# madsjulia/GeostatInversion.jl

Hardware: AMD Instinct MI355X
Metric: randSVD GB/s + top-k singular-value rel-err, n=1e6 rank=256 (higher is better)
Workload: dtype f64

## Files before the change

geostatinversion.jl_amd/_lib.py:

```python
import ctypes as C
import os

import numpy as np

_HERE = os.path.dirname(os.path.abspath(__file__))
LIB_PATH = os.path.join(_HERE, "libgsi_hip.so")

GSI_OK = 0
ERR_NAMES = {1: "GSI_ERR_ARG", 2: "GSI_ERR_NEG_ITERS", 3: "GSI_ERR_SINGULAR", 4: "GSI_ERR_HIP",
             5: "GSI_ERR_RCCL", 6: "GSI_ERR_OOM", 7: "GSI_ERR_NOT_POSDEF", 8: "GSI_ERR_INTERNAL"}
PHASES = ["gemm_n", "gemm_t", "lu", "qr", "svd", "small_gemm", "comm", "other", "comm_wait"]
UNIQUE_ID_BYTES = 128

c_i64 = C.c_int64
c_dp = C.POINTER(C.c_double)
c_vp = C.c_void_p
RANDN_FN = C.CFUNCTYPE(None, c_vp, c_dp, c_i64)

SIGNATURES = {
    "gsi_version": (C.c_int, []),
    "gsi_last_error": (C.c_char_p, []),
    "gsi_backend_name": (C.c_char_p, []),
    "gsi_ctx_create": (C.c_int, [C.POINTER(c_vp), C.c_int]),
    "gsi_ctx_destroy": (C.c_int, [c_vp]),
# ... 28 lines not shown
    "gsi_randsvd": (C.c_int, [c_vp, c_vp, c_dp, c_i64, c_i64, c_i64, c_dp, c_dp]),
    "gsi_randsvd_dense_host": (C.c_int, [c_vp, c_dp, c_i64, c_i64, c_i64, c_dp, c_i64, c_i64, c_i64, c_dp, c_dp, C.POINTER(c_vp)]),
    "gsi_rangefinder_dense_host": (C.c_int, [c_vp, c_dp, c_i64, c_i64, c_i64, c_dp, c_i64, c_i64, c_dp, C.POINTER(c_vp)]),
    "gsi_eig_nystrom": (C.c_int, [c_vp, c_vp, c_dp, c_i64, c_dp, c_dp]),
    "gsi_rangefinder_adaptive": (C.c_int, [c_vp, c_vp, RANDN_FN, c_vp, C.c_double, c_i64, c_dp, C.POINTER(c_i64)]),
    "gsi_mat_create": (C.c_int, [c_vp, C.POINTER(c_vp), c_i64, c_i64]),
    "gsi_mat_destroy": (C.c_int, [c_vp]),
    "gsi_mat_upload": (C.c_int, [c_vp, c_vp, c_dp, c_i64]),
    "gsi_mat_download": (C.c_int, [c_vp, c_vp, c_dp, c_i64]),
    "gsi_mat_randn": (C.c_int, [c_vp, c_vp, C.c_uint64]),
    "gsi_op_mul_dev": (C.c_int, [c_vp, c_vp, C.c_int, c_vp, c_vp]),
    "gsi_rangefinder_dev": (C.c_int, [c_vp, c_vp, c_vp, c_i64, c_vp]),
    "gsi_randsvd_dev": (C.c_int, [c_vp, c_vp, c_vp, c_i64, c_i64, c_i64, c_vp, c_vp]),
    "gsi_randsvd_rows": (C.c_int, [c_vp, c_vp, c_vp, c_i64, c_i64, c_i64, c_vp, c_vp]),
    "gsi_lu_L": (C.c_int, [c_vp, c_dp, c_i64, c_i64, c_dp, C.POINTER(C.c_int32)]),
    "gsi_lu_L_dev": (C.c_int, [c_vp, c_vp, C.POINTER(C.c_int32)]),
    "gsi_lu_L_sharded": (C.c_int, [c_vp, c_dp, c_i64, c_i64, c_dp, C.POINTER(C.c_int32)]),
    "gsi_lu_L_sharded_virtual": (C.c_int, [c_vp, c_dp, c_i64, c_i64, C.c_int, c_dp, C.POINTER(C.c_int32)]),
    "gsi_qr_thinQ": (C.c_int, [c_vp, c_dp, c_i64, c_i64, c_dp, c_dp]),
    "gsi_svd_tall": (C.c_int, [c_vp, c_dp, c_i64, c_i64, c_dp, c_dp]),
    "gsi_gemm": (C.c_int, [c_vp, C.c_int, c_i64, c_i64, c_i64, C.c_double, c_dp, c_i64, c_dp, c_i64, c_dp, c_i64]),
    "gsi_gemm_view": (C.c_int, [c_vp, C.c_int, C.c_int, c_i64, c_i64, c_i64, C.c_double, C.c_double, c_dp, c_i64, c_i64,
                                c_dp, c_i64, c_i64, c_dp, c_i64, c_i64, c_i64, c_i64, C.POINTER(c_i64)]),
    "gsi_pcga_params": (C.c_int, [c_vp, c_dp, c_i64, c_i64, c_dp, c_dp, C.c_double, c_dp]),
    "gsi_pcga_update": (C.c_int, [c_vp, c_dp, c_i64, c_i64, c_dp, C.c_double, c_dp, c_i64, c_dp, c_dp]),
    "gsi_pcga_params_dev": (C.c_int, [c_vp, c_vp, c_i64, c_dp, c_dp, C.c_double, c_dp]),
    "gsi_pcga_update_dev": (C.c_int, [c_vp, c_vp, c_i64, c_dp, C.c_double, c_dp, c_i64, c_dp, c_dp]),
    "gsi_mat_download_col": (C.c_int, [c_vp, c_vp, c_i64, c_dp]),
    "gsi_op_lowrank_solve": (C.c_int, [c_vp, c_vp, c_dp, c_dp, C.POINTER(c_i64)]),
    "gsi_pcgamat_create": (C.c_int, [c_vp, C.POINTER(c_vp), c_dp, c_i64, c_i64, c_dp, c_dp, C.c_int]),
    "gsi_pcgamat_destroy": (C.c_int, [c_vp]),
    "gsi_pcgamat_mul": (C.c_int, [c_vp, c_vp, c_dp, c_dp]),
    "gsi_pcgamat_lsqr": (C.c_int, [c_vp, c_vp, c_dp, c_dp, C.POINTER(c_i64)]),
    "gsi_basis_create": (C.c_int, [c_vp, C.POINTER(c_vp), c_vp, c_i64, C.c_int]),
    "gsi_basis_destroy": (C.c_int, [c_vp]),
    "gsi_pcga_params_basis": (C.c_int, [c_vp, c_vp, c_dp, c_dp, C.c_double, c_dp]),
    "gsi_pcga_update_basis": (C.c_int, [c_vp, c_vp, c_dp, C.c_double, c_dp, c_i64, c_dp, c_dp]),
    "gsi_basis_download_col": (C.c_int, [c_vp, c_vp, c_i64, c_dp]),
    "gsi_ctx_profile": (C.c_int, [c_vp, C.c_int]),
    "gsi_ctx_phase_reset": (C.c_int, [c_vp]),
    "gsi_ctx_phase_times": (C.c_int, [c_vp, c_dp, C.POINTER(c_i64)]),
    "gsi_ctx_counters": (C.c_int, [c_vp, C.POINTER(c_i64)]),
    "gsi_ctx_path_info": (C.c_int, [c_vp, C.POINTER(c_i64), c_i64]),
    "gsi_ctx_pinned_copy_rate": (C.c_int, [c_vp, c_i64, c_dp, c_dp]),
    "gsi_ctx_release_cache": (C.c_int, [c_vp]),
    "gsi_ctx_device_bytes": (C.c_int, [c_vp, C.POINTER(c_i64)]),
# ... 50 lines not shown
```

geostatinversion.jl_amd/csrc/api.cpp:

```cpp
#include <cmath>
#include <cstdlib>
#include <cstring>
#include <memory>
#include <new>
#include <string>
#include <vector>
#include "../../include/gsi_hip.h"
#include "pipeline.hpp"
#include "pointcov.hpp"

using namespace gsi;

struct gsi_ctx {
  Context c;
};
struct gsi_op {
  Operator op;
};
struct gsi_mat {
  gsi_ctx* ctx;
  Buf buf;
  int64_t rows, cols;
  int refs = 1;
};
// ... 944 lines not shown
    REQUIRE(form != 1 || m == l, "gemm_view: form 1 is the l x l product A'A (m == l)");
    REQUIRE(form != 3 || (r0 >= 0 && r0 + m <= m_full), "gemm_view: row block outside the full product");
    const bool tn = trans || form == 1;
    const int64_t ar = (form == 3) ? m_full : (tn ? k : m), ac = tn ? m : k;
    const int64_t crows = (form == 3) ? m_full : m;
    REQUIRE(lda >= ar && ldc >= crows && (form == 1 || ldb >= k), "leading dimension too small");
    REQUIRE(a_off >= 0 && b_off >= 0 && c_off >= 0, "negative offset");
    Backend* be = ctx->c.be.get();
    const size_t na = (size_t)a_off + (size_t)lda * (size_t)ac, nc = (size_t)c_off + (size_t)ldc * (size_t)l;
    const size_t nb = (form == 1) ? 1 : (size_t)b_off + (size_t)ldb * (size_t)l;
    Buf Ad(be, na), Bd(be, nb), Cd(be, nc);
    be->fill_bytes(Ad.p, 0xFF, na);
    be->fill_bytes(Bd.p, 0xFF, nb);
    be->upload2d(Ad.p + a_off, lda, A, ar, ar, ac);
    if (form != 1) be->upload2d(Bd.p + b_off, ldb, B, k, k, l);
    be->upload2d(Cd.p, (int64_t)nc, C, (int64_t)nc, (int64_t)nc, 1);
    be->gemm_view(form, trans != 0, m, l, k, alpha, Ad.p + a_off, lda, Bd.p + b_off, ldb, beta, Cd.p + c_off, ldc, m_full, r0,
                  plan_out);
    be->download2d(C, (int64_t)nc, Cd.p, (int64_t)nc, (int64_t)nc, 1);
    check_async_errors(ctx->c);
  });
}

namespace {
void pcga_params_impl(Context& c, const double* Zdev, int64_t n, int64_t K, const double* s, const double* X,
                      double delta, double* out) {
  Backend* be = c.be.get();
  Buf O(be, (size_t)n * (K + 3)), sv(be, (size_t)n), Xv(be, (size_t)n);
  be->upload2d(sv.p, n, s, n, n, 1);
  be->upload2d(Xv.p, n, X, n, n, 1);
  be->pcga_params(Zdev, n, K, sv.p, Xv.p, delta, O.p);
  be->download2d(out, n, O.p, n, n, K + 3);
}
void pcga_update_impl(Context& c, const double* Zdev, int64_t n, int64_t K, const double* X, double beta_bar,
                      const double* etas, int64_t nobs, const double* xi_bar, double* s_out) {
  Backend* be = c.be.get();
  Buf E(be, (size_t)nobs * K), xb(be, (size_t)nobs), w(be, (size_t)K), sd(be, (size_t)n), Xd(be, (size_t)n);
  be->upload2d(E.p, nobs, etas, nobs, nobs, K);
  be->upload2d(xb.p, nobs, xi_bar, nobs, nobs, 1);
  be->upload2d(Xd.p, n, X, n, n, 1);
  be->gemm_tn(K, 1, nobs, 1.0, E.p, nobs, xb.p, nobs, 0.0, w.p, K);
  be->scal_copy(n, beta_bar, Xd.p, sd.p);
  be->gemm_nn(n, 1, K, 1.0, Zdev, n, w.p, K, 1.0, sd.p, n);
  be->download2d(s_out, n, sd.p, n, n, 1);
}
}
// ... 246 lines not shown
```

geostatinversion.jl_amd/csrc/backend.hpp:

```cpp
#pragma once
#include <cstddef>
#include <cstdint>
#include <stdexcept>
#include <string>

namespace gsi {

struct Error : std::runtime_error {
  int code;
  Error(int c, const std::string& msg) : std::runtime_error(msg), code(c) {}
};

enum Phase : int {
  PH_GEMM_N = 0, PH_GEMM_T = 1, PH_LU = 2, PH_QR = 3, PH_SVD = 4, PH_SMALL_GEMM = 5,
  PH_COMM = 6, PH_OTHER = 7, PH_COMM_WAIT = 8, PH_COUNT = 9
};

class Backend {
 public:
  virtual ~Backend() {}
  virtual const char* name() const = 0;

  virtual double* alloc(size_t count) = 0;
  virtual void release(double* p) = 0;
// ... 11 lines not shown
    upload2d(dst, ldd, host, ldh, rows, cols);
    return nullptr;
  }
  virtual void pinned_copy_rate(int64_t bytes, double* h2d_gbs, double* d2h_gbs) { (void)bytes; *h2d_gbs = 0.0; *d2h_gbs = 0.0; }
  virtual void upload2d_wait_block(void* handle, int64_t b) { (void)handle; (void)b; }
  virtual void upload2d_end(void* handle) { (void)handle; }

  virtual void gemm_nn(int64_t m, int64_t l, int64_t k, double alpha, const double* A, int64_t lda,
                       const double* B, int64_t ldb, double beta, double* C, int64_t ldc) = 0;
  virtual void gemm_nn_rowblock(int64_t m_full, int64_t r0, int64_t mb, int64_t l, int64_t k, const double* A, int64_t lda,
                                const double* B, int64_t ldb, double* C, int64_t ldc) {
    (void)m_full;
    gemm_nn(mb, l, k, 1.0, A + r0, lda, B, ldb, 0.0, C + r0, ldc);
  }
  virtual void gemm_tn(int64_t m, int64_t l, int64_t k, double alpha, const double* A, int64_t lda,
                       const double* B, int64_t ldb, double beta, double* C, int64_t ldc) = 0;

  virtual void gemm_view(int form, bool trans, int64_t m, int64_t l, int64_t k, double alpha, const double* A, int64_t lda,
                         const double* B, int64_t ldb, double beta, double* C, int64_t ldc, int64_t m_full, int64_t r0,
                         int64_t* plan8) {
    (void)form; (void)trans; (void)m; (void)l; (void)k; (void)alpha; (void)A; (void)lda; (void)B; (void)ldb; (void)beta;
    (void)C; (void)ldc; (void)m_full; (void)r0; (void)plan8;
    throw Error(1 , "gemm_view: not available on this backend");
  }
  virtual void fill_bytes(double* p, int byte, size_t count) {
    (void)p; (void)byte; (void)count;
    throw Error(1 , "fill_bytes: not available on this backend");
  }

  virtual void gemm_nn_gridcov(int64_t m, int64_t l, int64_t k, const double* tab, int64_t nx, int64_t ny,
                               int64_t roff, int64_t koff, const double* B, int64_t ldb, double* C,
                               int64_t ldc) = 0;

  virtual void gemm_nn_pointcov(int64_t m, int64_t l, int64_t k, const double* pts, int d, int kind, double ell,
                                double sigma2, double nugget, int64_t roff, int64_t koff, const double* B, int64_t ldb,
                                double* C, int64_t ldc) = 0;

  virtual void* fftcov_create(const int64_t N[3], double beta, int fftrf) = 0;
  virtual void* fftcov_create_lags(const int64_t N[3], int kind, const double ell[3], double theta, double sigma2,
                                   double nugget, const double* table, const double* table_mirror) {
    (void)N; (void)kind; (void)ell; (void)theta; (void)sigma2; (void)nugget; (void)table; (void)table_mirror;
    throw Error(1 , "fft covariance from a covariance function or table: not supported by this backend");
  }
  virtual void fftcov_destroy(void* plan) = 0;
  virtual void fftcov_apply(void* plan, int64_t l, const double* X, int64_t ldx, double* Y, int64_t ldy) = 0;

// ... 170 lines not shown
```

geostatinversion.jl_amd/csrc/cholqr.hip:

```cpp
#include "hip_common.hpp"
#include <atomic>
#include <cfloat>
#include <cstdio>
#include <cstdlib>

namespace gsi { namespace hipk {

constexpr int CQ_TB = 32;

__global__ __launch_bounds__(256) void cq_diagmax_kernel(const double* __restrict__ G, int l, double* __restrict__ tiny) {
  __shared__ double s[256];
  double mx = 0.0;
  for (int i = threadIdx.x; i < l; i += 256) mx = fmax(mx, G[i + (int64_t)i * l]);
  s[threadIdx.x] = mx;
  __syncthreads();
  for (int st = 128; st > 0; st >>= 1) {
    if (threadIdx.x < st) s[threadIdx.x] = fmax(s[threadIdx.x], s[threadIdx.x + st]);
    __syncthreads();
  }
  if (threadIdx.x == 0) tiny[0] = s[0] * (double)l * DBL_EPSILON * 16.0;
}

__device__ __forceinline__ double cq_bcast(double v, int src) {
  const int lo = __builtin_amdgcn_readlane(__double2loint(v), src);
// ... 205 lines not shown
    for (int j = 0; j < 8; ++j) {
#pragma unroll
      for (int i = 0; i < j; ++i) acc[j] -= Ds[(pb + i) * CQF_DS + pb + j] * acc[i];
      acc[j] *= Dinv[pb + j];
    }
#pragma unroll
    for (int j = 0; j < 8; ++j) {
      const double v = (pb + j < b) ? acc[j] : 0.0;
      us[(pb + j) * CQF_LDU] = v;
      if constexpr (!VEC) { if (pb + j < b) gcol[pb + j] = v; }
    }
    if constexpr (VEC) {
      double2* o2 = reinterpret_cast<double2*>(gcol + pb);
#pragma unroll
      for (int j = 0; j < 8; j += 2) o2[j >> 1] = make_double2(acc[j], acc[j + 1]);
    }
    asm volatile("" ::: "memory");
  }
}
#define CQF_STAMP(ph) do { if (trace != nullptr && tid == 0) { const unsigned long long now_ = wall_clock64(); trace[ph] += now_ - t_last; t_last = now_; } } while (0)
__device__ __forceinline__ void cqf_tri_inverse(const double* __restrict__ G, int l, double* __restrict__ X, double* Us,
                                                double* Ds, int tid, int lane, int wave, unsigned long long* trace,
                                                unsigned long long& t_last);
__global__ __launch_bounds__(CQF_THREADS) void cq_chol_inv_kernel(double* __restrict__ G, int l, double* __restrict__ X,
                                                                  int32_t* __restrict__ flag, unsigned long long* __restrict__ trace) {
  unsigned long long t_last = (trace != nullptr) ? wall_clock64() : 0ull;
  extern __shared__ double cqf_lds[];
  double* Us = cqf_lds;
  double* Ds = Us + CQ_TB * CQF_LDU;
  double* Dinv = Ds + CQ_TB * CQF_DS;
  double* red = Dinv + CQ_TB;
  const int tid = threadIdx.x, lane = tid & 63, wave = tid >> 6;
  const int nblk = (l + CQ_TB - 1) / CQ_TB;
  {
    double mx = 0.0;
    for (int i = tid; i < l; i += CQF_THREADS) mx = fmax(mx, G[i + (int64_t)i * l]);
    for (int off = 32; off > 0; off >>= 1) mx = fmax(mx, __shfl_xor(mx, off, 64));
    if (lane == 0) red[wave] = mx;
    __syncthreads();
    if (tid == 0) {
      double m2 = 0.0;
      for (int w2 = 0; w2 < CQF_THREADS / 64; ++w2) m2 = fmax(m2, red[w2]);
      red[32] = m2 * (double)l * DBL_EPSILON * 16.0;
    }
    for (int64_t e = tid; e < (int64_t)l * l; e += CQF_THREADS) X[e] = 0.0;
    __syncthreads();
  }
  const double tiny = red[32];
  CQF_STAMP(0);

  auto trailing_tiles = [&](int j0, int b, int nc, int ncp, bool first_rows, int w0, int nw) __attribute__((always_inline)) {
    const int nt = ncp >> 4;
    const int nfirst = (nt >= 2) ? (2 * nt - 1) : nt;
    const int ntot = nt * (nt + 1) / 2;
    const int cnt = first_rows ? nfirst : ntot - nfirst;
    const int base = first_rows ? 0 : nfirst;
    const int jl = lane & 15, kq = lane >> 4;
    double* Gt = G + (int64_t)(j0 + b) + (int64_t)(j0 + b) * l;
    constexpr int TPP = 4;
    if (wave < w0 || wave >= w0 + nw) return;
    for (int t0 = wave - w0; t0 < cnt; t0 += nw * TPP) {
      cq_double4 acc[TPP];
      int trs[TPP], tcs[TPP];
#pragma unroll
      for (int u = 0; u < TPP; ++u) {
        const int tl = t0 + u * nw;
        int tr = 0, rem = base + ((tl < cnt) ? tl : 0);
        while (rem >= nt - tr) { rem -= nt - tr; ++tr; }
// ... 42 lines not shown
        else cqf_block_row_col<false>(G + j0 + (int64_t)(j0 + b + c) * l, b, Ds, Dinv, Us + c);
      } else {
#pragma unroll
        for (int p = 0; p < CQ_TB; ++p) Us[p * CQF_LDU + c] = 0.0;
      }
    }
    for (int e = tid; e < b * nc; e += CQF_THREADS) {
      const int r = j0 + b + e % nc, c = j0 + e / nc;
      G[r + (int64_t)c * l] = 0.0;
    }
    __syncthreads();
    CQF_STAMP(2);
    trailing_tiles(j0, b, nc, ncp, true, 0, CQF_THREADS / 64);
    __syncthreads();
    {
      const int j1 = j0 + b;
      const int b1 = (l - j1 < CQ_TB) ? (l - j1) : CQ_TB;
      if (wave == 0) cqf_chol_diag(G, l, j1, b1, tiny, Ds, Dinv, flag, lane);
      trailing_tiles(j0, b, nc, ncp, false, 1, CQF_THREADS / 64 - 1);
    }
    __syncthreads();
    CQF_STAMP(3);
  }
  cqf_tri_inverse(G, l, X, Us, Ds, tid, lane, wave, trace, t_last);
}

__device__ __forceinline__ void cqf_tri_inverse(const double* __restrict__ G, int l, double* __restrict__ X, double* Us,
                                                double* Ds, int tid, int lane, int wave, unsigned long long* trace,
                                                unsigned long long& t_last) {
  const int nblk = (l + CQ_TB - 1) / CQ_TB;
  for (int jb = wave; jb < nblk; jb += CQF_THREADS / 64) {
    const int j0 = jb * CQ_TB;
    cqf_inv_diag(G, l, j0, (l - j0 < CQ_TB) ? (l - j0) : CQ_TB, X, lane);
  }
  __syncthreads();
  CQF_STAMP(4);
  double* Wt = Us;
  double* Xjj = Ds;
  for (int jb = 1; jb < nblk; ++jb) {
    const int j0 = jb * CQ_TB;
    const int b = (l - j0 < CQ_TB) ? (l - j0) : CQ_TB;
    for (int e = tid; e < CQ_TB * CQ_TB; e += CQF_THREADS) {
      const int r = e & (CQ_TB - 1), c = e >> 5;
      Xjj[r * CQF_DS + c] = (r < b && c < b) ? X[(j0 + r) + (int64_t)(j0 + c) * l] : 0.0;
    }
    __syncthreads();
    {
// ... 181 lines not shown
  const int l = (int)l64;
  const CqBufs b = cq_bufs(small, l);
  if (!trmm_upper_tall(st, m, l, T, ldt, b.X2, l, Y, ld)) gemm_f64_trmm_upper(st, m, l, l, T, ldt, b.X2, l, Y, ld, gemm_ws);
  if (R != nullptr)
    hipLaunchKernelGGL(cq_triprod_kernel, dim3(grid_for((int64_t)l * l, 256)), dim3(256), 0, st, b.R2, b.R1, l, R);
}

void cholqr2_R(hipStream_t st, int64_t l64, double* small, double* R) {
  const int l = (int)l64;
  const CqBufs b = cq_bufs(small, l);
  hipLaunchKernelGGL(cq_triprod_kernel, dim3(grid_for((int64_t)l * l, 256)), dim3(256), 0, st, b.R2, b.R1, l, R);
}
const double* cholqr2_X2(const double* small, int64_t l) { return small + 5 * (size_t)l * (size_t)l; }

void mirror_upper(hipStream_t st, double* G, int64_t l) {
  hipLaunchKernelGGL(cq_mirror_upper_kernel, dim3(64), dim3(256), 0, st, G, (int)l);
}
bool cq_gram_round(hipStream_t st, double* Gm, int64_t l64, double* X, bool check, int32_t* flag) {
  const int l = (int)l64;
  if (l < 1 || l > CQF_MAXL) return false;
  hipLaunchKernelGGL(cq_mirror_upper_kernel, dim3(64), dim3(256), 0, st, Gm, l);
  if (check)
    hipLaunchKernelGGL(cq_orth_check_kernel, dim3(grid_for((int64_t)l * l, 64)), dim3(256), 0, st, Gm, l, 0.1, flag);
  static std::atomic<uint64_t> attr_mask{0};
  if (first_use_on_this_device(attr_mask))
    (void)hipFuncSetAttribute((const void*)cq_chol_inv_kernel, hipFuncAttributeMaxDynamicSharedMemorySize, (int)CQF_LDS_BYTES);
  hipLaunchKernelGGL(cq_chol_inv_kernel, dim3(1), dim3(CQF_THREADS), CQF_LDS_BYTES, st, Gm, l, X, flag,
                     (unsigned long long*)nullptr);
  return true;
}
void tri_product(hipStream_t st, const double* R2, const double* R1, int64_t l, double* R) {
  hipLaunchKernelGGL(cq_triprod_kernel, dim3(grid_for(l * l, 256)), dim3(256), 0, st, R2, R1, (int)l, R);
}

__global__ __launch_bounds__(256) void lr_gather_rows_kernel(const double* __restrict__ S, int64_t lds, int64_t N,
                                                             const int64_t* __restrict__ src, const int64_t* __restrict__ sub,
                                                             int64_t nr, double* __restrict__ R, int64_t ldr) {
  const int64_t total = nr * N;
  for (int64_t e = (int64_t)blockIdx.x * blockDim.x + threadIdx.x; e < total; e += (int64_t)gridDim.x * blockDim.x) {
    const int64_t k = e % nr, c = e / nr;
    const double* col = S + c * lds;
    const int64_t s = sub[k];
    double v = col[src[k]];
    if (s >= 0) v -= col[s];
    R[k + c * ldr] = v;
  }
// ... 60 lines not shown
```

geostatinversion.jl_amd/csrc/hip_backend.hip:

```cpp
#include <hip/hip_runtime.h>
#include <rccl/rccl.h>
#include <dlfcn.h>
#include <fcntl.h>
#include <sched.h>
#include <sys/mman.h>
#include <time.h>
#include <unistd.h>
#include <algorithm>
#include <cmath>
#include <cstdlib>
#include <cstring>
#include <condition_variable>
#include <atomic>
#include <mutex>
#include <string>
#include <chrono>
#include <map>
#include <memory>
#include <set>
#include <vector>
#include "../../include/gsi_hip.h"
#include "backend.hpp"
#include "hip_common.hpp"
#include "host_staging.hpp"
// ... 311 lines not shown
    check_launch("gemm_tn");
  }
  void gemm_view(int form, bool trans, int64_t m, int64_t l, int64_t k, double alpha, const double* A, int64_t lda,
                 const double* B, int64_t ldb, double beta, double* C, int64_t ldc, int64_t m_full, int64_t r0,
                 int64_t* plan8) override {
    bind();
    hipk::GemmPlan p = {0, 0, 0, 0, 0, 0, 0, 0};
    if (form == 0) {
      double* ws = gemm_ws(hipk::gemm_workspace_doubles(m, l, k));
      hipk::gemm_f64(st_, trans, m, l, k, alpha, A, lda, B, ldb, beta, C, ldc, ws, &p);
    } else if (form == 1) {
      double* ws = gemm_ws(hipk::gemm_syrk_workspace_doubles(l, k));
      hipk::gemm_f64_syrk_upper(st_, l, k, A, lda, C, ldc, ws, &p);
    } else if (form == 2) {
      double* ws = gemm_ws(hipk::gemm_workspace_doubles(m, l, k));
      hipk::gemm_f64_trmm_upper(st_, m, l, k, A, lda, B, ldb, C, ldc, ws, &p);
    } else {
      double* ws = gemm_ws(hipk::gemm_rowblock_workspace_doubles(m_full, m, l, k));
      hipk::gemm_f64_nn_rowblock(st_, m_full, r0, m, l, k, A, lda, B, ldb, C, ldc, ws, &p);
    }
    check_launch("gemm_view");
    const int64_t out[8] = {p.nt, p.nchunks, p.xmode, p.wide, p.nsplit, p.persistent, p.grid_x, p.active};
    for (int i = 0; i < 8; ++i) plan8[i] = out[i];
  }
  void fill_bytes(double* p, int byte, size_t count) override {
    bind();
    HIP_CHECK(hipMemsetAsync(p, byte, count * sizeof(double), st_));
  }
  void gemm_nn_gridcov(int64_t m, int64_t l, int64_t k, const double* tab, int64_t nx, int64_t ny, int64_t roff,
                       int64_t koff, const double* B, int64_t ldb, double* C, int64_t ldc) override {
    bind();
    double* ws = gemm_ws(hipk::gemm_workspace_doubles(m, l, k));
    hipk::gemm_f64_gridcov(st_, m, l, k, tab, nx, ny, roff, koff, B, ldb, C, ldc, ws);
    check_launch("gemm_nn_gridcov");
  }

  void gemm_nn_pointcov(int64_t m, int64_t l, int64_t k, const double* pts, int d, int kind, double ell, double sigma2,
                        double nugget, int64_t roff, int64_t koff, const double* B, int64_t ldb, double* C,
                        int64_t ldc) override {
    bind();
    if (m <= 0 || l <= 0 || k <= 0) return;
    const int64_t npts = std::max(roff + m, koff + k);
    Scratch p4(this, (size_t)4 * npts);
    hipk::pointcov_pad_points(st_, pts, d, npts, hipk::pointcov_point_scale(kind, 1.0 / ell), p4.p);
    double* ws = gemm_ws(hipk::gemm_pointcov_workspace_doubles(m, l, k));
    double* xpack = nullptr;
// ... 556 lines not shown
    bind();
    static const bool off = (getenv("GSI_NO_CHOLQR") != nullptr);
    if (off || l < 1 || l > 384 || l > N - 1 || K < 1 || K > l || N > 4096 || n < 2 * l) return false;
    const size_t Nl = ((size_t)N * l + 7) & ~(size_t)7, ll = ((size_t)l * l + 7) & ~(size_t)7;
    Scratch buf(this, 3 * Nl + 12 * ll);
    double* A0 = buf.p;
    double* A1 = A0 + Nl;
    double* P = A1 + Nl;
    double* Gr[4];
    for (int i = 0; i < 4; ++i) Gr[i] = P + Nl + (size_t)i * ll;
    double* X[4];
    for (int i = 0; i < 4; ++i) X[i] = P + Nl + (size_t)(4 + i) * ll;
    double* R = P + Nl + 8 * ll;
    double* Rf = R + ll;
    double* U = Rf + ll;
    double* Mm = U + ll;
    size_t gmax = hipk::gemm_workspace_doubles(N, l, N);
    gmax = std::max(gmax, hipk::gemm_workspace_doubles(l, l, N));
    gmax = std::max(gmax, hipk::gemm_workspace_doubles(N, l, l));
    gmax = std::max(gmax, hipk::gemm_workspace_doubles(l, l, l));
    gmax = std::max(gmax, hipk::gemm_workspace_doubles(N, K, l));
    gmax = std::max(gmax, hipk::gemm_workspace_doubles(n, K, N));
    double* ws = gemm_ws(gmax + 64);
    auto round = [&](const double* M, int i, bool check) {
      hipk::gemm_f64(st_, false, N, l, N, 1.0, G, N, M, N, 0.0, P, N, ws);
      hipk::gemm_f64(st_, true, l, l, N, 1.0, M, N, P, N, 0.0, Gr[i], l, ws);
      (void)hipk::cq_gram_round(st_, Gr[i], l, X[i], check, flags_ + 9);
    };
    int32_t f = 0;
    phase_begin(PH_QR);
    HIP_CHECK(hipMemsetAsync(flags_ + 9, 0, sizeof(int32_t), st_));
    hipk::scal_copy(st_, (int64_t)N * l, c, T, A0);
    round(A0, 0, false);
    hipk::gemm_f64(st_, false, N, l, l, 1.0, A0, N, X[0], l, 0.0, A1, N, ws);
    round(A1, 1, true);
    hipk::scal_copy(st_, (int64_t)N * l, c, P, A0);
    round(A0, 2, false);
    hipk::gemm_f64(st_, false, N, l, l, 1.0, A0, N, X[2], l, 0.0, A1, N, ws);
    round(A1, 3, true);
    check_launch("lowrank_tail");
    HIP_CHECK(hipMemcpyAsync(&f, flags_ + 9, sizeof(int32_t), hipMemcpyDeviceToHost, st_));
    HIP_CHECK(hipStreamSynchronize(st_));
    if (f != 0) {
      phase_end(PH_QR);
      return false;
    }
    hipk::tri_product(st_, Gr[3], Gr[2], l, R);
    hipk::gemm_f64(st_, false, l, l, l, 1.0, R, l, X[1], l, 0.0, Rf, l, ws);
    phase_end(PH_QR);
    n_cholqr_ += 2;
    phase_begin(PH_SVD);
    svd_small(Rf, l, U, Sv);
    hipk::scale_cols_sqrt(st_, U, l, Sv, K);
    phase_end(PH_SVD);
    phase_begin(PH_SMALL_GEMM);
    hipk::gemm_f64(st_, false, l, K, l, 1.0, X[3], l, U, l, 0.0, Mm, l, ws);
    hipk::gemm_f64(st_, false, N, K, l, 1.0, A1, N, Mm, l, 0.0, A0, N, ws);
    hipk::gemm_f64(st_, false, n, K, N, 1.0, Sm, lds, A0, N, 0.0, Z, ldz, ws);
    if (K < l) HIP_CHECK(hipMemsetAsync(Z + (size_t)K * ldz, 0, sizeof(double) * ((size_t)(l - K - 1) * ldz + n), st_));
    check_launch("lowrank_tail");
    phase_end(PH_SMALL_GEMM);
    return true;
  }
  bool lowrank_power_step(const double* Sm, int64_t lds, int64_t n, int64_t N, const double* G, const double* T,
                          const int32_t* ipiv, const double* L, int64_t ldl, int64_t l, double c, double* Tn) override {
    bind();
    static const bool trace = (getenv("GSI_LOWRANK_POWER_TRACE") != nullptr);
    constexpr int64_t NSAMPLE = 256;
    constexpr int NPARTS = 128;
    constexpr double CHECK_MAX = 1e-8;
    if (l < 1 || l > 384 || N < 1 || N > 4096 || n < 2 * l || n >= ((int64_t)1 << 31)) return false;
    const int64_t ns = std::min<int64_t>(NSAMPLE, n - l), nchk = l + ns;
    auto up8 = [](int64_t x) { return (x + 7) & ~(int64_t)7; };
    const int64_t o_chk = up8(2 * l), o_sm = o_chk + up8(nchk), nr = o_sm + 2 * l, ldr = up8(nr);
    const size_t nidx = (size_t)(2 * ldr + nchk);
    const size_t ll = (size_t)up8(l * l), Nl = (size_t)up8(N * l);
    Scratch buf(this, 2 * ll + Nl + (size_t)ldr * (size_t)N + (size_t)ldr * (size_t)l + nidx + NPARTS + 2);
    double* Mp = buf.p;
    double* Ut = Mp + ll;
    double* C = Ut + ll;
    double* R = C + Nl;
    double* E = R + (size_t)ldr * N;
    int64_t* idx_dev = reinterpret_cast<int64_t*>(E + (size_t)ldr * l);
    double* part = reinterpret_cast<double*>(idx_dev + nidx);
// ... 944 lines not shown
```

geostatinversion.jl_amd/csrc/hip_common.hpp:

```cpp
#pragma once
#include <hip/hip_runtime.h>
#include <atomic>
#include <cstdint>
#include <cstddef>
#include "pointcov.hpp"

namespace gsi { namespace hipk {

inline bool first_use_on_this_device(std::atomic<uint64_t>& mask) {
  int dev = 0;
  if (hipGetDevice(&dev) != hipSuccess || dev < 0 || dev > 63) return true;
  const uint64_t bit = (uint64_t)1 << dev;
  return (mask.fetch_or(bit, std::memory_order_acq_rel) & bit) == 0;
}

struct GemmPlan { int64_t nt, nchunks, xmode, wide, nsplit, persistent, grid_x, active; };
size_t gemm_workspace_doubles(int64_t M, int64_t L, int64_t K);
void gemm_f64(hipStream_t st, bool transA, int64_t M, int64_t L, int64_t K, double alpha, const double* A,
              int64_t lda, const double* B, int64_t ldb, double beta, double* C, int64_t ldc, double* ws,
              GemmPlan* plan = nullptr);
size_t gemm_rowblock_workspace_doubles(int64_t M_full, int64_t mb, int64_t L, int64_t K);
void gemm_f64_nn_rowblock(hipStream_t st, int64_t M_full, int64_t r0, int64_t mb, int64_t L, int64_t K, const double* A,
                          int64_t lda, const double* B, int64_t ldb, double* C, int64_t ldc, double* ws,
                          GemmPlan* plan = nullptr);
// ... 136 lines not shown
void cholqr2_factor(hipStream_t st, const double* Y, int64_t m, int64_t l, int64_t ld, double* T, int64_t ldt,
                    double* small_ws, int32_t* flag, double* gemm_ws);
void cholqr2_apply(hipStream_t st, double* Y, int64_t m, int64_t l, int64_t ld, const double* T, int64_t ldt,
                   double* R, double* small_ws, double* gemm_ws);
void cholqr2_R(hipStream_t st, int64_t l, double* small_ws, double* R);
const double* cholqr2_X2(const double* small_ws, int64_t l);
void mirror_upper(hipStream_t st, double* G, int64_t l);
bool cq_gram_round(hipStream_t st, double* Gm, int64_t l, double* X, bool check, int32_t* flag);
void tri_product(hipStream_t st, const double* R2, const double* R1, int64_t l, double* R);
bool tri_inverse(hipStream_t st, const double* R, int64_t l, double* X);
void lr_gather_rows(hipStream_t st, const double* S, int64_t lds, int64_t N, const int64_t* src, const int64_t* sub,
                    int64_t nr, double* R, int64_t ldr);
void lr_check_rows(hipStream_t st, const double* E, int64_t lde, const double* L, int64_t ldl, const int64_t* rows,
                   int64_t nchk, int64_t l, double* part, int nparts);
void scholqr3_factor(hipStream_t st, const double* Y, int64_t m, int64_t l, int64_t ld, double* T, int64_t ldt,
                     double* S, int64_t lds, double* small_ws, int32_t* flag, double* gemm_ws);
void scholqr3_apply(hipStream_t st, double* Y, int64_t m, int64_t l, int64_t ld, const double* S, int64_t lds,
                    double* R, double* small_ws, double* gemm_ws);

void lr_compose(hipStream_t st, const int32_t* piv, const int32_t* info, int64_t n, int64_t l, int64_t nchk, int64_t o_chk,
                int64_t o_sm, int64_t ldr, int64_t* src, int64_t* sub, int64_t* chk, int32_t* verdict);
void lr_solve_u(hipStream_t st, const double* L, int64_t ldl, const double* Mp, int64_t l, double c, double* Ut);
void lr_solve_c(hipStream_t st, const double* Ut, int64_t l, const double* T, int64_t N, double c, double* C);
void lr_solve_u12(hipStream_t st, const double* L, int64_t ldl, const double* Mp, int64_t l1, int64_t l, double c, double* Ut11,
                  double* U12);
void lr_move_rows(hipStream_t st, double* X, int64_t ldx, int64_t nc, const int64_t* src, const int64_t* sub,
                  const int32_t* verdict, int64_t maxmv, double* tmp, int64_t ldt, int64_t nzero);
void lr_pivots(hipStream_t st, const int32_t* piv, int64_t cnt, int64_t add, int32_t* dst);
void lr_forget_zero_pivot(hipStream_t st, int32_t* info);
struct SvdWork {
  int32_t* rotcount;
  double* norms;
  int32_t* pairs;
};
constexpr int SVD_SCHED_INTS = 4096;
int svd_small(hipStream_t st, double* G, int64_t l, double* U, double* S, const SvdWork& w);

void center_rows(hipStream_t st, double* S, int64_t n, int64_t N, int64_t ld);
void scale_cols_sqrt(hipStream_t st, double* U, int64_t l, const double* S, int64_t K);
void randn_fill(hipStream_t st, double* p, size_t count, uint64_t seed);
void fill_gridcov(hipStream_t st, double* A, int64_t lda, int64_t nx, int64_t ny, double ell, int kind,
                  int64_t row0, int64_t mloc);
void fill_lowrank_samples(hipStream_t st, double* S, int64_t ld, int64_t nloc, int64_t N, int64_t row0, uint64_t seed,
                          double decay);
void colnorms_sq(hipStream_t st, const double* Y, int64_t m, int64_t c, int64_t ld, double* out_dev);
void chol_upper(hipStream_t st, double* B, int64_t j, int32_t* info);
// ... 23 lines not shown
```

geostatinversion.jl_amd/csrc/lowrank_power.hip:

```cpp
#include "hip_common.hpp"
#include <climits>

namespace gsi { namespace hipk {

constexpr int LRP_MAXL = 384;
constexpr int LRP_THREADS = 256;
constexpr int LRP_ITEMS = 3;

constexpr int LRP_PER = (LRP_MAXL + LRP_THREADS - 1) / LRP_THREADS;

__global__ __launch_bounds__(LRP_THREADS) void lr_compose_kernel(const int32_t* __restrict__ piv, const int32_t* __restrict__ info,
                                                                 int64_t n, int l, int nchk, int64_t o_chk, int64_t o_sm,
                                                                 int64_t ldr, int64_t* __restrict__ src, int64_t* __restrict__ sub,
                                                                 int64_t* __restrict__ chk, int32_t* __restrict__ verdict) {
  __shared__ int32_t top[LRP_MAXL], pv[LRP_MAXL], up[LRP_MAXL], lk[LRP_MAXL], lv[LRP_MAXL], sk[LRP_MAXL], sv[LRP_MAXL];
  __shared__ int32_t scan[LRP_THREADS];
  __shared__ int32_t cnt_s, bad_s;
  const int tid = threadIdx.x;
  if (tid == 0) { cnt_s = 0; bad_s = 0; }
  __syncthreads();
  for (int j = tid; j < l; j += LRP_THREADS) {
    int64_t r = piv[j];
    if (r < j || r >= n) { bad_s = 1; r = r < j ? j : n - 1; }
    pv[j] = (int32_t)r;
// ... 226 lines not shown
#pragma unroll
  for (int cc = 0; cc < NC; ++cc)
#pragma unroll
    for (int ib = 0; ib < LRP_MAXL / 64; ++ib) xs[cc][ib * 64 + lane] = v[cc][ib];
  __syncthreads();
  lrp_lower_solve<NC, false>(Ut, l, l, xs, lane);
  for (int cc = 0; cc < NC; ++cc) {
    if (r0 + cc >= N) break;
    for (int i = lane; i < l; i += 64) C[r0 + cc + (int64_t)i * N] = c * xs[cc][i];
  }
}

constexpr int LRP_NC_U = 2, LRP_NC_C = 4;

void lr_solve_u(hipStream_t st, const double* L, int64_t ldl, const double* Mp, int64_t l, double c, double* Ut) {
  hipLaunchKernelGGL(lr_solve_u_kernel<LRP_NC_U>, dim3((unsigned)((l + LRP_NC_U - 1) / LRP_NC_U)), dim3(64), 0, st, L, ldl, Mp,
                     (int)l, c, Ut);
}
void lr_solve_c(hipStream_t st, const double* Ut, int64_t l, const double* T, int64_t N, double c, double* C) {
  hipLaunchKernelGGL(lr_solve_c_kernel<LRP_NC_C>, dim3((unsigned)((N + LRP_NC_C - 1) / LRP_NC_C)), dim3(64), 0, st, Ut, (int)l, T,
                     N, c, C);
}

template <int NC>
__global__ __launch_bounds__(64) void lr_solve_u12_kernel(const double* __restrict__ L, int64_t ldl, const double* __restrict__ Mp,
                                                          int l1, int l, double c, double* __restrict__ Ut11,
                                                          double* __restrict__ U12) {
  __shared__ double xs[NC][LRP_MAXL];
  const int lane = threadIdx.x, col0 = blockIdx.x * NC;
  const int m = (col0 + NC < l1) ? col0 + NC : l1;
  double v[NC][LRP_MAXL / 64];
#pragma unroll
  for (int cc = 0; cc < NC; ++cc)
#pragma unroll
    for (int ib = 0; ib < LRP_MAXL / 64; ++ib) {
      const int i = ib * 64 + lane;
      v[cc][ib] = (i < m && col0 + cc < l) ? Mp[i + (int64_t)(col0 + cc) * l1] : 0.0;
    }
  __builtin_amdgcn_sched_barrier(0);
#pragma unroll
  for (int cc = 0; cc < NC; ++cc)
#pragma unroll
    for (int ib = 0; ib < LRP_MAXL / 64; ++ib) xs[cc][ib * 64 + lane] = v[cc][ib];
  __syncthreads();
  lrp_lower_solve<NC, true>(L, ldl, m, xs, lane);
  for (int cc = 0; cc < NC; ++cc) {
// ... 69 lines not shown
```

include/gsi_hip.h:

```cpp
#ifndef GSI_HIP_H
#define GSI_HIP_H

#include <stdint.h>

#ifdef __cplusplus
extern "C" {
#endif

#define GSI_VERSION 100

#define GSI_OK 0
#define GSI_ERR_ARG 1
#define GSI_ERR_NEG_ITERS 2
#define GSI_ERR_SINGULAR 3
#define GSI_ERR_HIP 4
#define GSI_ERR_RCCL 5
#define GSI_ERR_OOM 6
#define GSI_ERR_NOT_POSDEF 7
#define GSI_ERR_INTERNAL 8

typedef struct gsi_ctx gsi_ctx;
typedef struct gsi_op gsi_op;
typedef struct gsi_mat gsi_mat;

// ... 79 lines not shown
int gsi_mat_download(gsi_ctx* ctx, const gsi_mat* mat, double* host, int64_t ldh);
int gsi_mat_randn(gsi_ctx* ctx, gsi_mat* mat, uint64_t seed);
int gsi_op_mul_dev(gsi_ctx* ctx, const gsi_op* op, int trans, const gsi_mat* X, gsi_mat* Y);
int gsi_rangefinder_dev(gsi_ctx* ctx, const gsi_op* op, const gsi_mat* Omega,
                        int64_t numiterations, gsi_mat* Q);
int gsi_randsvd_dev(gsi_ctx* ctx, const gsi_op* op, const gsi_mat* Omega, int64_t K, int64_t p,
                    int64_t q, gsi_mat* Z, gsi_mat* S);

int gsi_randsvd_rows(gsi_ctx* ctx, const gsi_op* op, const gsi_mat* Omega_rows, int64_t K, int64_t p, int64_t q,
                     gsi_mat* Z_rows, gsi_mat* S);

int gsi_lu_L(gsi_ctx* ctx, const double* Y, int64_t m, int64_t l, double* L_out, int32_t* ipiv_out);
int gsi_lu_L_dev(gsi_ctx* ctx, gsi_mat* Y, int32_t* ipiv_out);
int gsi_lu_L_sharded(gsi_ctx* ctx, const double* Y, int64_t m, int64_t l, double* L_out, int32_t* ipiv_out);
int gsi_lu_L_sharded_virtual(gsi_ctx* ctx, const double* Y, int64_t m, int64_t l, int nshards, double* L_out,
                             int32_t* ipiv_out);
int gsi_qr_thinQ(gsi_ctx* ctx, const double* Y, int64_t m, int64_t l, double* Q_out, double* R_out);
int gsi_svd_tall(gsi_ctx* ctx, const double* W, int64_t n, int64_t l, double* V_out, double* S_out);
int gsi_gemm(gsi_ctx* ctx, int trans, int64_t m, int64_t l, int64_t k, double alpha,
             const double* A, int64_t lda, const double* B, int64_t ldb, double* C, int64_t ldc);
int gsi_gemm_view(gsi_ctx* ctx, int form, int trans, int64_t m, int64_t l, int64_t k, double alpha, double beta,
                  const double* A, int64_t lda, int64_t a_off, const double* B, int64_t ldb, int64_t b_off,
                  double* C, int64_t ldc, int64_t c_off, int64_t m_full, int64_t r0, int64_t* plan_out);

int gsi_pcga_params(gsi_ctx* ctx, const double* Z, int64_t n, int64_t K, const double* s,
                    const double* X, double delta, double* out);
int gsi_pcga_update(gsi_ctx* ctx, const double* Z, int64_t n, int64_t K, const double* X,
                    double beta_bar, const double* etas, int64_t nobs, const double* xi_bar,
                    double* s_out);

int gsi_pcga_params_dev(gsi_ctx* ctx, const gsi_mat* basis, int64_t K, const double* s, const double* X,
                        double delta, double* out);
int gsi_pcga_update_dev(gsi_ctx* ctx, const gsi_mat* basis, int64_t K, const double* X, double beta_bar,
                        const double* etas, int64_t nobs, const double* xi_bar, double* s_out);
int gsi_mat_download_col(gsi_ctx* ctx, const gsi_mat* mat, int64_t col, double* host);

int gsi_op_lowrank_solve(gsi_ctx* ctx, const gsi_op* op, const double* b, double* x_out, int64_t* iters_out);

typedef struct gsi_pcgamat gsi_pcgamat;
int gsi_pcgamat_create(gsi_ctx* ctx, gsi_pcgamat** mat, const double* etas, int64_t nobs, int64_t K, const double* HX,
                       const double* R, int r_is_diag);
int gsi_pcgamat_destroy(gsi_pcgamat* mat);
int gsi_pcgamat_mul(gsi_ctx* ctx, const gsi_pcgamat* mat, const double* x, double* y);
int gsi_pcgamat_lsqr(gsi_ctx* ctx, const gsi_pcgamat* mat, const double* b, double* x_out, int64_t* iters_out);

typedef struct gsi_basis gsi_basis;
// ... 47 lines not shown
```

Before: 1711.

## Replace triangular inverses with triangular solves in low-rank CholQR tail

The low-rank randSVD tail no longer forms explicit inverses of the Cholesky factors. Applying R^{-1} now goes through new right and left upper-triangular solve kernels instead of GEMMs with the inverted factor, and a Cholesky-only kernel variant is launched. The mid-tail host flag readback and stream sync are moved to the end, so the SVD and small GEMMs are queued without a host round trip; sweep counters are restored if the flag reports failure. This drops the inverse kernel and one synchronization in exchange for a serial solve kernel with limited parallelism, and adds a test entry point plus an env var that restores the old inverse path.

Result: no change. 1722 (median of 6 runs) (+0.6%).

```diff
diff --git a/geostatinversion.jl_amd/_lib.py b/geostatinversion.jl_amd/_lib.py
--- a/geostatinversion.jl_amd/_lib.py
+++ b/geostatinversion.jl_amd/_lib.py
@@ -74,6 +74,7 @@
     "gsi_gemm": (C.c_int, [c_vp, C.c_int, c_i64, c_i64, c_i64, C.c_double, c_dp, c_i64, c_dp, c_i64, c_dp, c_i64]),
     "gsi_gemm_view": (C.c_int, [c_vp, C.c_int, C.c_int, c_i64, c_i64, c_i64, C.c_double, C.c_double, c_dp, c_i64, c_i64,
                                 c_dp, c_i64, c_i64, c_dp, c_i64, c_i64, c_i64, c_i64, C.POINTER(c_i64)]),
+    "gsi_tail_solve_view": (C.c_int, [c_vp, C.c_int, c_i64, c_i64, c_dp, c_dp, c_dp, c_i64, c_i64, C.POINTER(C.c_int32)]),
     "gsi_pcga_params": (C.c_int, [c_vp, c_dp, c_i64, c_i64, c_dp, c_dp, C.c_double, c_dp]),
     "gsi_pcga_update": (C.c_int, [c_vp, c_dp, c_i64, c_i64, c_dp, C.c_double, c_dp, c_i64, c_dp, c_dp]),
     "gsi_pcga_params_dev": (C.c_int, [c_vp, c_vp, c_i64, c_dp, c_dp, C.c_double, c_dp]),
diff --git a/geostatinversion.jl_amd/csrc/api.cpp b/geostatinversion.jl_amd/csrc/api.cpp
--- a/geostatinversion.jl_amd/csrc/api.cpp
+++ b/geostatinversion.jl_amd/csrc/api.cpp
@@ -990,6 +990,30 @@
   });
 }
 
+int gsi_tail_solve_view(gsi_ctx* ctx, int op, int64_t l, int64_t rows, const double* R, const double* B, double* X_image,
+                        int64_t x_off, int64_t x_len, int32_t* flag_out) {
+  return guarded([&] {
+    REQUIRE(ctx && X_image && flag_out, "NULL argument");
+    REQUIRE(op >= 0 && op <= 3, "tail_solve_view: op is 0 (factor), 1 (factor and inverse), 2 (right solve) or 3 (left solve)");
+    REQUIRE(l >= 1 && l <= 384 && rows >= 1, "tail_solve_view: need 1 <= l <= 384, rows >= 1");
+    REQUIRE(op < 2 || (R && B), "NULL argument");
+    REQUIRE(op != 3 || rows <= l, "tail_solve_view: the left solve takes at most l columns");
+    const int64_t outc = (op < 2) ? l * l : rows * l;
+    REQUIRE(x_off >= 0 && x_off + outc <= x_len, "tail_solve_view: the output does not fit its image");
+    Backend* be = ctx->c.be.get();
+    const int64_t brows = (op == 2) ? rows : l;
+    Buf Xd(be, (size_t)x_len), Rd(be, op < 2 ? 1 : (size_t)l * l), Bd(be, op < 2 ? 1 : (size_t)brows * l);
+    be->upload2d(Xd.p, x_len, X_image, x_len, x_len, 1);
+    if (op >= 2) {
+      be->upload2d(Rd.p, l, R, l, l, l);
+      be->upload2d(Bd.p, brows, B, brows, brows, l);
+    }
+    be->tail_solve_view(op, l, rows, Rd.p, Bd.p, Xd.p + x_off, flag_out);
+    be->download2d(X_image, x_len, Xd.p, x_len, x_len, 1);
+    check_async_errors(ctx->c);
+  });
+}
+
 namespace {
 void pcga_params_impl(Context& c, const double* Zdev, int64_t n, int64_t K, const double* s, const double* X,
                       double delta, double* out) {
diff --git a/geostatinversion.jl_amd/csrc/backend.hpp b/geostatinversion.jl_amd/csrc/backend.hpp
--- a/geostatinversion.jl_amd/csrc/backend.hpp
+++ b/geostatinversion.jl_amd/csrc/backend.hpp
@@ -57,6 +57,10 @@
     (void)form; (void)trans; (void)m; (void)l; (void)k; (void)alpha; (void)A; (void)lda; (void)B; (void)ldb; (void)beta;
     (void)C; (void)ldc; (void)m_full; (void)r0; (void)plan8;
     throw Error(1 , "gemm_view: not available on this backend");
+  }
+  virtual void tail_solve_view(int op, int64_t l, int64_t rows, const double* R, const double* B, double* X, int32_t* flag) {
+    (void)op; (void)l; (void)rows; (void)R; (void)B; (void)X; (void)flag;
+    throw Error(1 , "tail_solve_view: not available on this backend");
   }
   virtual void fill_bytes(double* p, int byte, size_t count) {
     (void)p; (void)byte; (void)count;
diff --git a/geostatinversion.jl_amd/csrc/cholqr.hip b/geostatinversion.jl_amd/csrc/cholqr.hip
--- a/geostatinversion.jl_amd/csrc/cholqr.hip
+++ b/geostatinversion.jl_amd/csrc/cholqr.hip
@@ -251,8 +251,9 @@
 __device__ __forceinline__ void cqf_tri_inverse(const double* __restrict__ G, int l, double* __restrict__ X, double* Us,
                                                 double* Ds, int tid, int lane, int wave, unsigned long long* trace,
                                                 unsigned long long& t_last);
-__global__ __launch_bounds__(CQF_THREADS) void cq_chol_inv_kernel(double* __restrict__ G, int l, double* __restrict__ X,
-                                                                  int32_t* __restrict__ flag, unsigned long long* __restrict__ trace) {
+template <bool INV>
+__device__ __forceinline__ void cqf_chol_body(double* __restrict__ G, int l, double* __restrict__ X, int32_t* __restrict__ flag,
+                                              unsigned long long* __restrict__ trace) {
   unsigned long long t_last = (trace != nullptr) ? wall_clock64() : 0ull;
   extern __shared__ double cqf_lds[];
   double* Us = cqf_lds;
@@ -272,7 +273,9 @@
       for (int w2 = 0; w2 < CQF_THREADS / 64; ++w2) m2 = fmax(m2, red[w2]);
       red[32] = m2 * (double)l * DBL_EPSILON * 16.0;
     }
-    for (int64_t e = tid; e < (int64_t)l * l; e += CQF_THREADS) X[e] = 0.0;
+    if constexpr (INV) {
+      for (int64_t e = tid; e < (int64_t)l * l; e += CQF_THREADS) X[e] = 0.0;
+    }
     __syncthreads();
   }
   const double tiny = red[32];
@@ -361,7 +364,14 @@
     __syncthreads();
     CQF_STAMP(3);
   }
-  cqf_tri_inverse(G, l, X, Us, Ds, tid, lane, wave, trace, t_last);
+  if constexpr (INV) cqf_tri_inverse(G, l, X, Us, Ds, tid, lane, wave, trace, t_last);
+}
+__global__ __launch_bounds__(CQF_THREADS) void cq_chol_inv_kernel(double* __restrict__ G, int l, double* __restrict__ X,
+                                                                  int32_t* __restrict__ flag, unsigned long long* __restrict__ trace) {
+  cqf_chol_body<true>(G, l, X, flag, trace);
+}
+__global__ __launch_bounds__(CQF_THREADS) void cq_chol_kernel(double* __restrict__ G, int l, int32_t* __restrict__ flag) {
+  cqf_chol_body<false>(G, l, nullptr, flag, nullptr);
 }
 
 __device__ __forceinline__ void cqf_tri_inverse(const double* __restrict__ G, int l, double* __restrict__ X, double* Us,
@@ -589,6 +599,13 @@
   hipLaunchKernelGGL(cq_mirror_upper_kernel, dim3(64), dim3(256), 0, st, Gm, l);
   if (check)
     hipLaunchKernelGGL(cq_orth_check_kernel, dim3(grid_for((int64_t)l * l, 64)), dim3(256), 0, st, Gm, l, 0.1, flag);
+  if (X == nullptr) {
+    static std::atomic<uint64_t> attr_mask_f{0};
+    if (first_use_on_this_device(attr_mask_f))
+      (void)hipFuncSetAttribute((const void*)cq_chol_kernel, hipFuncAttributeMaxDynamicSharedMemorySize, (int)CQF_LDS_BYTES);
+    hipLaunchKernelGGL(cq_chol_kernel, dim3(1), dim3(CQF_THREADS), CQF_LDS_BYTES, st, Gm, l, flag);
+    return true;
+  }
   static std::atomic<uint64_t> attr_mask{0};
   if (first_use_on_this_device(attr_mask))
     (void)hipFuncSetAttribute((const void*)cq_chol_inv_kernel, hipFuncAttributeMaxDynamicSharedMemorySize, (int)CQF_LDS_BYTES);
diff --git a/geostatinversion.jl_amd/csrc/hip_backend.hip b/geostatinversion.jl_amd/csrc/hip_backend.hip
--- a/geostatinversion.jl_amd/csrc/hip_backend.hip
+++ b/geostatinversion.jl_amd/csrc/hip_backend.hip
@@ -357,6 +357,25 @@
     check_launch("gemm_view");
     const int64_t out[8] = {p.nt, p.nchunks, p.xmode, p.wide, p.nsplit, p.persistent, p.grid_x, p.active};
     for (int i = 0; i < 8; ++i) plan8[i] = out[i];
+  }
+  void tail_solve_view(int op, int64_t l, int64_t rows, const double* R, const double* B, double* X, int32_t* flag) override {
+    bind();
+    int32_t f = 0;
+    if (op == 0 || op == 1) {
+      Scratch inv(this, op == 1 ? (size_t)l * l : 0);
+      HIP_CHECK(hipMemsetAsync(flags_ + 9, 0, sizeof(int32_t), st_));
+      if (!hipk::cq_gram_round(st_, X, l, op == 1 ? inv.p : nullptr, false, flags_ + 9))
+        throw Error(GSI_ERR_ARG, "tail_solve_view: l beyond the fused Cholesky kernel");
+      HIP_CHECK(hipMemcpyAsync(&f, flags_ + 9, sizeof(int32_t), hipMemcpyDeviceToHost, st_));
+    } else if (op == 2) {
+      Scratch ut(this, (size_t)l * l);
+      hipk::lr_solve_right_upper(st_, R, l, B, rows, ut.p, X);
+    } else {
+      hipk::lr_solve_left_upper(st_, R, l, B, rows, X);
+    }
+    check_launch("tail_solve_view");
+    HIP_CHECK(hipStreamSynchronize(st_));
+    *flag = f;
   }
   void fill_bytes(double* p, int byte, size_t count) override {
     bind();
@@ -959,44 +978,53 @@
     gmax = std::max(gmax, hipk::gemm_workspace_doubles(N, K, l));
     gmax = std::max(gmax, hipk::gemm_workspace_doubles(n, K, N));
     double* ws = gemm_ws(gmax + 64);
+    static const bool inverses = (getenv("GSI_TAIL_INVERSES") != nullptr);
     auto round = [&](const double* M, int i, bool check) {
       hipk::gemm_f64(st_, false, N, l, N, 1.0, G, N, M, N, 0.0, P, N, ws);
       hipk::gemm_f64(st_, true, l, l, N, 1.0, M, N, P, N, 0.0, Gr[i], l, ws);
-      (void)hipk::cq_gram_round(st_, Gr[i], l, X[i], check, flags_ + 9);
+      (void)hipk::cq_gram_round(st_, Gr[i], l, inverses ? X[i] : nullptr, check, flags_ + 9);
+    };
+    auto unround = [&](const double* B, int64_t rows, int i, double* D) {
+      if (inverses) hipk::gemm_f64(st_, false, rows, l, l, 1.0, B, rows, X[i], l, 0.0, D, rows, ws);
+      else hipk::lr_solve_right_upper(st_, Gr[i], l, B, rows, X[i], D);
     };
     int32_t f = 0;
+    const int sweeps_before = last_svd_sweeps_;
+    const int64_t cap_hits_before = n_svd_cap_hits_;
     phase_begin(PH_QR);
     HIP_CHECK(hipMemsetAsync(flags_ + 9, 0, sizeof(int32_t), st_));
     hipk::scal_copy(st_, (int64_t)N * l, c, T, A0);
     round(A0, 0, false);
-    hipk::gemm_f64(st_, false, N, l, l, 1.0, A0, N, X[0], l, 0.0, A1, N, ws);
+    unround(A0, N, 0, A1);
     round(A1, 1, true);
     hipk::scal_copy(st_, (int64_t)N * l, c, P, A0);
     round(A0, 2, false);
-    hipk::gemm_f64(st_, false, N, l, l, 1.0, A0, N, X[2], l, 0.0, A1, N, ws);
+    unround(A0, N, 2, A1);
     round(A1, 3, true);
+    hipk::tri_product(st_, Gr[3], Gr[2], l, R);
+    unround(R, l, 1, Rf);
     check_launch("lowrank_tail");
-    HIP_CHECK(hipMemcpyAsync(&f, flags_ + 9, sizeof(int32_t), hipMemcpyDeviceToHost, st_));
-    HIP_CHECK(hipStreamSynchronize(st_));
-    if (f != 0) {
-      phase_end(PH_QR);
-      return false;
-    }
-    hipk::tri_product(st_, Gr[3], Gr[2], l, R);
-    hipk::gemm_f64(st_, false, l, l, l, 1.0, R, l, X[1], l, 0.0, Rf, l, ws);
     phase_end(PH_QR);
-    n_cholqr_ += 2;
     phase_begin(PH_SVD);
     svd_small(Rf, l, U, Sv);
     hipk::scale_cols_sqrt(st_, U, l, Sv, K);
     phase_end(PH_SVD);
     phase_begin(PH_SMALL_GEMM);
-    hipk::gemm_f64(st_, false, l, K, l, 1.0, X[3], l, U, l, 0.0, Mm, l, ws);
+    if (inverses) hipk::gemm_f64(st_, false, l, K, l, 1.0, X[3], l, U, l, 0.0, Mm, l, ws);
+    else hipk::lr_solve_left_upper(st_, Gr[3], l, U, K, Mm);
     hipk::gemm_f64(st_, false, N, K, l, 1.0, A1, N, Mm, l, 0.0, A0, N, ws);
     hipk::gemm_f64(st_, false, n, K, N, 1.0, Sm, lds, A0, N, 0.0, Z, ldz, ws);
     if (K < l) HIP_CHECK(hipMemsetAsync(Z + (size_t)K * ldz, 0, sizeof(double) * ((size_t)(l - K - 1) * ldz + n), st_));
     check_launch("lowrank_tail");
     phase_end(PH_SMALL_GEMM);
+    HIP_CHECK(hipMemcpyAsync(&f, flags_ + 9, sizeof(int32_t), hipMemcpyDeviceToHost, st_));
+    HIP_CHECK(hipStreamSynchronize(st_));
+    if (f != 0) {
+      last_svd_sweeps_ = sweeps_before;
+      n_svd_cap_hits_ = cap_hits_before;
+      return false;
+    }
+    n_cholqr_ += 2;
     return true;
   }
   bool lowrank_power_step(const double* Sm, int64_t lds, int64_t n, int64_t N, const double* G, const double* T,
diff --git a/geostatinversion.jl_amd/csrc/hip_common.hpp b/geostatinversion.jl_amd/csrc/hip_common.hpp
--- a/geostatinversion.jl_amd/csrc/hip_common.hpp
+++ b/geostatinversion.jl_amd/csrc/hip_common.hpp
@@ -182,6 +182,8 @@
                 int64_t o_sm, int64_t ldr, int64_t* src, int64_t* sub, int64_t* chk, int32_t* verdict);
 void lr_solve_u(hipStream_t st, const double* L, int64_t ldl, const double* Mp, int64_t l, double c, double* Ut);
 void lr_solve_c(hipStream_t st, const double* Ut, int64_t l, const double* T, int64_t N, double c, double* C);
+void lr_solve_right_upper(hipStream_t st, const double* R, int64_t l, const double* B, int64_t N, double* Ut, double* X);
+void lr_solve_left_upper(hipStream_t st, const double* R, int64_t l, const double* B, int64_t K, double* X);
 void lr_solve_u12(hipStream_t st, const double* L, int64_t ldl, const double* Mp, int64_t l1, int64_t l, double c, double* Ut11,
                   double* U12);
 void lr_move_rows(hipStream_t st, double* X, int64_t ldx, int64_t nc, const int64_t* src, const int64_t* sub,
diff --git a/geostatinversion.jl_amd/csrc/lowrank_power.hip b/geostatinversion.jl_amd/csrc/lowrank_power.hip
--- a/geostatinversion.jl_amd/csrc/lowrank_power.hip
+++ b/geostatinversion.jl_amd/csrc/lowrank_power.hip
@@ -272,6 +272,112 @@
                      N, c, C);
 }
 
+__global__ __launch_bounds__(256) void lr_transpose_kernel(const double* __restrict__ R, int l, double* __restrict__ Ut) {
+  __shared__ double t[32][33];
+  const int bx = blockIdx.x * 32, by = blockIdx.y * 32, tx = threadIdx.x & 31, ty = threadIdx.x >> 5;
+  for (int j = ty; j < 32; j += 8) {
+    const int r = bx + tx, c = by + j;
+    t[j][tx] = (r < l && c < l) ? R[r + (int64_t)c * l] : 0.0;
+  }
+  __syncthreads();
+  for (int j = ty; j < 32; j += 8) {
+    const int r = by + tx, c = bx + j;
+    if (r < l && c < l) Ut[r + (int64_t)c * l] = t[tx][j];
+  }
+}
+
+template <int NC>
+__device__ __forceinline__ void lrp_upper_solve(const double* __restrict__ M, int64_t ldm, int m, double (*xs)[LRP_MAXL],
+                                                int lane) {
+  const int nb = (m + 63) >> 6;
+  for (int t = nb - 1; t >= 0; --t) {
+    const int row = t * 64 + lane;
+    const int rowc = row < m ? row : m - 1;
+    const double* __restrict__ Mr = M + rowc;
+    double acc[NC];
+#pragma unroll
+    for (int c = 0; c < NC; ++c) acc[c] = xs[c][rowc];
+    for (int j0 = (t + 1) * 64; j0 < nb * 64; j0 += 64) {
+      double a[64];
+#pragma unroll
+      for (int u = 0; u < 64; ++u) {
+        const int col = j0 + u;
+        a[u] = col < m ? Mr[(int64_t)col * ldm] : 0.0;
+      }
+      __builtin_amdgcn_sched_barrier(0);
+#pragma unroll
+      for (int u = 0; u < 64; ++u)
+#pragma unroll
+        for (int c = 0; c < NC; ++c) acc[c] = fma(-a[u], xs[c][j0 + u], acc[c]);
+    }
+    double a[64];
+#pragma unroll
+    for (int u = 0; u < 64; ++u) {
+      const int col = t * 64 + u;
+      a[u] = Mr[(int64_t)(col < m ? col : m - 1) * ldm];
+    }
+    const double d = M[rowc + (int64_t)rowc * ldm];
+    __builtin_amdgcn_sched_barrier(0);
+    const double rd = 1.0 / d;
+#pragma unroll
+    for (int c = 0; c < NC; ++c) acc[c] *= rd;
+#pragma unroll
+    for (int u = 0; u < 64; ++u) a[u] *= rd;
+#pragma unroll
+    for (int u = 0; u < 64; ++u) a[u] = (rowc < t * 64 + u && t * 64 + u < m) ? a[u] : 0.0;
+#pragma unroll
+    for (int u = 63; u >= 0; --u)
+#pragma unroll
+      for (int c = 0; c < NC; ++c) acc[c] = fma(-a[u], lrp_readlane(acc[c], u), acc[c]);
+    if (row < m) {
+#pragma unroll
+      for (int c = 0; c < NC; ++c) xs[c][row] = acc[c];
+    }
+    __syncthreads();
+  }
+}
+
+template <int NC>
+__global__ __launch_bounds__(64) void lr_solve_l_kernel(const double* __restrict__ R, int l, const double* __restrict__ B, int K,
+                                                        double* __restrict__ X) {
+  __shared__ double xs[NC][LRP_MAXL];
+  const int lane = threadIdx.x, col0 = blockIdx.x * NC;
+  double v[NC][LRP_MAXL / 64];
+#pragma unroll
+  for (int cc = 0; cc < NC; ++cc)
+#pragma unroll
+    for (int ib = 0; ib < LRP_MAXL / 64; ++ib) {
+      const int i = ib * 64 + lane;
+      v[cc][ib] = (i < l && col0 + cc < K) ? B[i + (int64_t)(col0 + cc) * l] : 0.0;
+    }
+  __builtin_amdgcn_sched_barrier(0);
+#pragma unroll
+  for (int cc = 0; cc < NC; ++cc)
+#pragma unroll
+    for (int ib = 0; ib < LRP_MAXL / 64; ++ib) xs[cc][ib * 64 + lane] = v[cc][ib];
+  __syncthreads();
+  lrp_upper_solve<NC>(R, l, l, xs, lane);
+  for (int cc = 0; cc < NC; ++cc) {
+    const int col = col0 + cc;
+    if (col >= K) break;
+    for (int i = lane; i < l; i += 64) X[i + (int64_t)col * l] = xs[cc][i];
+  }
+}
+
+constexpr int LRP_NC_L = 2;
+
+void lr_solve_right_upper(hipStream_t st, const double* R, int64_t l, const double* B, int64_t N, double* Ut, double* X) {
+  if (l < 1 || l > LRP_MAXL || N < 1) return;
+  const unsigned g = (unsigned)((l + 31) / 32);
+  hipLaunchKernelGGL(lr_transpose_kernel, dim3(g, g), dim3(256), 0, st, R, (int)l, Ut);
+  lr_solve_c(st, Ut, l, B, N, 1.0, X);
+}
+void lr_solve_left_upper(hipStream_t st, const double* R, int64_t l, const double* B, int64_t K, double* X) {
+  if (l < 1 || l > LRP_MAXL || K < 1) return;
+  hipLaunchKernelGGL(lr_solve_l_kernel<LRP_NC_L>, dim3((unsigned)((K + LRP_NC_L - 1) / LRP_NC_L)), dim3(64), 0, st, R, (int)l, B,
+                     (int)K, X);
+}
+
 template <int NC>
 __global__ __launch_bounds__(64) void lr_solve_u12_kernel(const double* __restrict__ L, int64_t ldl, const double* __restrict__ Mp,
                                                           int l1, int l, double c, double* __restrict__ Ut11,
diff --git a/include/gsi_hip.h b/include/gsi_hip.h
--- a/include/gsi_hip.h
+++ b/include/gsi_hip.h
@@ -125,6 +125,8 @@
 int gsi_gemm_view(gsi_ctx* ctx, int form, int trans, int64_t m, int64_t l, int64_t k, double alpha, double beta,
                   const double* A, int64_t lda, int64_t a_off, const double* B, int64_t ldb, int64_t b_off,
                   double* C, int64_t ldc, int64_t c_off, int64_t m_full, int64_t r0, int64_t* plan_out);
+int gsi_tail_solve_view(gsi_ctx* ctx, int op, int64_t l, int64_t rows, const double* R, const double* B, double* X_image,
+                        int64_t x_off, int64_t x_len, int32_t* flag_out);
 
 int gsi_pcga_params(gsi_ctx* ctx, const double* Z, int64_t n, int64_t K, const double* s,
                     const double* X, double delta, double* out);
```
